# ZhenghaoFei/visual_odom

Measured on NVIDIA H100. Metric: stereo frames/sec at 1241x376, 2000 feats; LK kernel HBM GB/s vs roofline, higher is better.
Workload: dtype u8/i32 fixed point + f32 (LK), f64 (pose)

## Files before the change

### visual_odom_b200/csrc/ctx.cu

```cuda
#include "ctx.h"
#include <string.h>
#include <stdlib.h>

void vo_set_error(vo_ctx* ctx, const char* fmt, ...)
{
    if (!ctx) return;
    va_list ap;
    va_start(ap, fmt);
    vsnprintf(ctx->err, sizeof(ctx->err), fmt, ap);
    va_end(ap);
}

extern "C" void vo_default_params(vo_params* p)
{
    p->fast_threshold = 20;
    p->fast_nonmax = 1;
    p->lk_win = 21;
    p->lk_max_level = 3;
    p->lk_max_iters = 30;
    p->lk_epsilon = 0.01;
    p->lk_min_eig = 0.001;
    p->circ_threshold = 0;
    p->pnp_iterations = 500;
    p->pnp_reproj_error = 0.5f;
// ... 255 lines not shown
}

typedef CUresult (*PFN_cuDeviceGet)(CUdevice*, int);
typedef CUresult (*PFN_cuDeviceGetDevResource)(CUdevice, CUdevResource*, CUdevResourceType);
typedef CUresult (*PFN_cuDevSmResourceSplitByCount)(CUdevResource*, unsigned int*, const CUdevResource*, CUdevResource*, unsigned int, unsigned int);
typedef CUresult (*PFN_cuDevResourceGenerateDesc)(CUdevResourceDesc*, CUdevResource*, unsigned int);
typedef CUresult (*PFN_cuGreenCtxCreate)(CUgreenCtx*, CUdevResourceDesc, CUdevice, unsigned int);
typedef CUresult (*PFN_cuGreenCtxStreamCreate)(CUstream*, CUgreenCtx, unsigned int, int);
typedef CUresult (*PFN_cuGreenCtxDestroy)(CUgreenCtx);

template <typename F>
static bool drv(const char* name, F* fn)
{
    void* p = nullptr;
    cudaDriverEntryPointQueryResult q;
    if (cudaGetDriverEntryPoint(name, &p, cudaEnableDefault, &q) != cudaSuccess || q != cudaDriverEntryPointSuccess || !p) return false;
    *fn = (F)p;
    return true;
}

void vo_partition_destroy(vo_ctx* ctx)
{
    for (auto& L : ctx->lane) {
        if (L.pre) cudaStreamDestroy(L.pre);
        if (L.post && L.post != L.pre) cudaStreamDestroy(L.post);
        L.pre = L.lk = L.post = nullptr;
    }
    PFN_cuGreenCtxDestroy destroy = nullptr;
    if (drv("cuGreenCtxDestroy", &destroy))
        for (int k = 0; k < 2; k++) if (ctx->part_gctx[k]) destroy((CUgreenCtx)ctx->part_gctx[k]);
    ctx->part_gctx[0] = ctx->part_gctx[1] = nullptr;
    ctx->part_on = false; ctx->part_helper_sms = ctx->part_lk_sms = 0;
}

int vo_partition_enable(vo_ctx* ctx, int helper_sms)
{
    VO_CUDA_CHECK(cudaSetDevice(ctx->device));
    int rc = vo_drain_pending(ctx);
    if (rc) return rc;
    VO_CUDA_CHECK(cudaDeviceSynchronize());
    vo_drop_graphs(ctx);
    vo_partition_destroy(ctx);
    if (helper_sms <= 0) return VO_OK;
    PFN_cuDeviceGet dget; PFN_cuDeviceGetDevResource getres; PFN_cuDevSmResourceSplitByCount split;
    PFN_cuDevResourceGenerateDesc gendesc; PFN_cuGreenCtxCreate create; PFN_cuGreenCtxStreamCreate screate;
    if (!drv("cuDeviceGet", &dget) || !drv("cuDeviceGetDevResource", &getres) || !drv("cuDevSmResourceSplitByCount", &split) ||
        !drv("cuDevResourceGenerateDesc", &gendesc) || !drv("cuGreenCtxCreate", &create) || !drv("cuGreenCtxStreamCreate", &screate)) {
        vo_set_error(ctx, "sm_partition: this driver has no green-context API");
        return VO_E_UNSUPPORTED;
    }
    CUdevice dev;
    CUdevResource all, part[1], rest;
    unsigned int nb = 1;
    CUresult r;
    if ((r = dget(&dev, ctx->device)) != CUDA_SUCCESS || (r = getres(dev, &all, CU_DEV_RESOURCE_TYPE_SM)) != CUDA_SUCCESS ||
        (r = split(part, &nb, &all, &rest, 0, (unsigned)helper_sms)) != CUDA_SUCCESS || nb != 1) {
        vo_set_error(ctx, "sm_partition: splitting off %d SMs failed (driver error %d)", helper_sms, (int)r);
        return VO_E_UNSUPPORTED;
    }
    CUdevResource* rs[2] = {&part[0], &rest};
    for (int k = 0; k < 2; k++) {
        CUdevResourceDesc desc;
        CUgreenCtx g;
        if ((r = gendesc(&desc, rs[k], 1)) != CUDA_SUCCESS || (r = create(&g, desc, dev, CU_GREEN_CTX_DEFAULT_STREAM)) != CUDA_SUCCESS) {
            vo_set_error(ctx, "sm_partition: cuGreenCtxCreate failed (driver error %d)", (int)r);
            vo_partition_destroy(ctx);
            return VO_E_UNSUPPORTED;
        }
        ctx->part_gctx[k] = g;
    }
    ctx->part_helper_sms = (int)part[0].sm.smCount; ctx->part_lk_sms = (int)rest.sm.smCount;
    for (int c = 0; c < VO_LANES; c++) {
        CUstream a, b;
        if ((r = screate(&a, (CUgreenCtx)ctx->part_gctx[0], CU_STREAM_NON_BLOCKING, 0)) != CUDA_SUCCESS ||
            (r = screate(&b, (CUgreenCtx)ctx->part_gctx[1], CU_STREAM_NON_BLOCKING, 0)) != CUDA_SUCCESS) {
            vo_set_error(ctx, "sm_partition: cuGreenCtxStreamCreate failed (driver error %d)", (int)r);
            vo_partition_destroy(ctx);
            return VO_E_UNSUPPORTED;
        }
        vo_ctx::Lane& L = ctx->lane[c];
        L.pre = L.lk = (cudaStream_t)b;
        L.post = (cudaStream_t)a;
    }
    ctx->part_on = true;
    return VO_OK;
}

int vo_drain_pending(vo_ctx* ctx)
{
    for (auto& p : ctx->pending)
        if (p.active) {
            VO_CUDA_CHECK(cudaEventSynchronize(p.done));
            p.active = false;
        }
    if (ctx->seq_inflight > 0 && ctx->lane[0].side) VO_CUDA_CHECK(cudaStreamSynchronize(ctx->lane[0].side));
    return VO_OK;
}

void vo_drop_graphs(vo_ctx* ctx)
{
    for (auto& g : ctx->graphs) cudaGraphExecDestroy(g.exec);
    ctx->graphs.clear();
}

static bool same_key(const GraphKey& a, const GraphKey& b)
{
    return a.kind == b.kind && a.s == b.s && a.tma == b.tma && a.u0 == b.u0 && a.n == b.n && a.max_pts == b.max_pts &&
           a.detect == b.detect && a.slot == b.slot && a.parity == b.parity && a.bgr == b.bgr;
}

int vo_run_graph(vo_ctx* ctx, const GraphKey& key, const std::function<int()>& launch)
{
    if (!ctx->use_graphs) return launch();
    for (auto& g : ctx->graphs)
        if (same_key(g.key, key)) {
            VO_CUDA_CHECK(cudaGraphLaunch(g.exec, key.s));
            ctx->launches += g.launches;
            return VO_OK;
        }
    const bool timing = ctx->lk_timing;
    const long long before = ctx->launches;
    ctx->lk_timing = false;
    cudaGraph_t graph = nullptr;
    VO_CUDA_CHECK(cudaStreamBeginCapture(key.s, cudaStreamCaptureModeThreadLocal));
    int rc = launch();
    cudaError_t e = cudaStreamEndCapture(key.s, &graph);
    ctx->lk_timing = timing;
    if (rc) { if (graph) cudaGraphDestroy(graph); return rc; }
    VO_CUDA_CHECK(e);
    vo_ctx::CachedGraph g;
    g.key = key;
    g.launches = ctx->launches - before;
    VO_CUDA_CHECK(cudaGraphInstantiate(&g.exec, graph, 0));
    cudaGraphDestroy(graph);
    ctx->graphs.push_back(g);
    VO_CUDA_CHECK(cudaGraphLaunch(g.exec, key.s));
    return VO_OK;
}

int vo_ensure_lanes(vo_ctx* ctx)
{
    if (ctx->fork_ev) return VO_OK;
    VO_CUDA_CHECK(cudaEventCreateWithFlags(&ctx->fork_ev, cudaEventDisableTiming));
    for (auto& L : ctx->lane) {
        VO_CUDA_CHECK(cudaStreamCreateWithFlags(&L.side, cudaStreamNonBlocking));
        VO_CUDA_CHECK(cudaEventCreateWithFlags(&L.join, cudaEventDisableTiming));
        for (cudaEvent_t& e : L.ev) VO_CUDA_CHECK(cudaEventCreateWithFlags(&e, cudaEventDisableTiming));
    }
    return VO_OK;
}

template <typename T>
static int write_table(vo_ctx* ctx, std::vector<T>& host, T* dev, int u0, int n, const T* e)
{
    const size_t e0 = (size_t)(1 + u0);
    if (memcmp(host.data() + e0, e, n * sizeof(T)) == 0) return VO_OK;
    memcpy(host.data() + e0, e, n * sizeof(T));
    for (auto& p : ctx->pending)
        if (p.active) VO_CUDA_CHECK(cudaStreamWaitEvent(ctx->stream, p.done, 0));
    VO_CUDA_CHECK(cudaMemcpyAsync(dev + e0, host.data() + e0, n * sizeof(T), cudaMemcpyHostToDevice, ctx->stream));
    return VO_OK;
}

int vo_write_calib(vo_ctx* ctx, int u0, int n, const CamCalib* c) { return write_table(ctx, ctx->cal, ctx->d_cal_tab, u0, n, c); }

int vo_write_params(vo_ctx* ctx, int u0, int n, const UnitParams* e) { return write_table(ctx, ctx->par, ctx->d_par_tab, u0, n, e); }

int vo_set_calibration(vo_ctx* ctx, int u0, int n, const float* P_l, const float* P_r, int n_mat)
{
    std::vector<CamCalib> c(n);
    for (int i = 0; i < n; i++) c[i] = vo_calib_from(P_l + 12 * (i % n_mat), P_r + 12 * (i % n_mat));
    return vo_write_calib(ctx, u0, n, c.data());
}

void vo_free_state(vo_ctx* ctx)
{
    vo_drop_graphs(ctx);
    for (void* p : ctx->allocs) cudaFree(p);
    ctx->allocs.clear();
    if (ctx->d_seq_state) cudaFree(ctx->d_seq_state);
    ctx->d_seq_state = nullptr; ctx->seq_n_cap = 0;
    ctx->d_feat_pts = nullptr; ctx->d_feat_ages = nullptr; ctx->d_feat_cnt = ctx->d_bucket = ctx->d_seq_err = ctx->d_seq_live = nullptr;
    ctx->d_out = nullptr; ctx->out_stride = 0; ctx->out_per = 0;
    ctx->d_cal_tab = ctx->d_cal = nullptr;
    ctx->d_par_tab = ctx->d_par = nullptr;
    ctx->d_geo = nullptr;
    ctx->w = ctx->h = ctx->units = 0;
}

template <typename T>
static cudaError_t dalloc(vo_ctx* ctx, T** p, size_t count)
{
    void* q = nullptr;
    cudaError_t e = cudaMalloc(&q, count * sizeof(T) + 256);
    if (e == cudaSuccess) { ctx->allocs.push_back(q); *p = (T*)q; }
    return e;
}

typedef CUresult (*PFN_encodeTiled)(CUtensorMap*, CUtensorMapDataType, cuuint32_t, void*, const cuuint64_t*,
                                    const cuuint64_t*, const cuuint32_t*, const cuuint32_t*, CUtensorMapInterleave,
                                    CUtensorMapSwizzle, CUtensorMapL2promotion, CUtensorMapFloatOOBfill);

static int encode_maps(vo_ctx* ctx)
{
    void* fn = nullptr;
    cudaDriverEntryPointQueryResult qres;
    VO_CUDA_CHECK(cudaGetDriverEntryPoint("cuTensorMapEncodeTiled", &fn, cudaEnableDefault, &qres));
    if (!fn || qres != cudaDriverEntryPointSuccess) {
        vo_set_error(ctx, "cuTensorMapEncodeTiled not available from the driver");
        return VO_E_CUDA;
    }
    PFN_encodeTiled enc = (PFN_encodeTiled)fn;
    const int n_img = ctx->units * 4;
    for (int l = 0; l < ctx->pg.nlevels; l++) {
        const LevelGeom& g = ctx->pg.lv[l];
        {
            cuuint64_t dims[3] = {(cuuint64_t)g.pitch, (cuuint64_t)g.hp, (cuuint64_t)n_img};
            cuuint64_t strides[2] = {(cuuint64_t)g.pitch, (cuuint64_t)g.plane};
            cuuint32_t box_i[3] = {48, 22, 1}, box_j[3] = {48, 32, 1};
            cuuint32_t estr[3] = {1, 1, 1};
            CUresult r = enc(&ctx->maps.img_i[l], CU_TENSOR_MAP_DATA_TYPE_UINT8, 3, g.img, dims, strides, box_i, estr,
                             CU_TENSOR_MAP_INTERLEAVE_NONE, CU_TENSOR_MAP_SWIZZLE_NONE,
                             CU_TENSOR_MAP_L2_PROMOTION_NONE, CU_TENSOR_MAP_FLOAT_OOB_FILL_NONE);
            if (r == CUDA_SUCCESS)
                r = enc(&ctx->maps.img_j[l], CU_TENSOR_MAP_DATA_TYPE_UINT8, 3, g.img, dims, strides, box_j, estr,
                        CU_TENSOR_MAP_INTERLEAVE_NONE, CU_TENSOR_MAP_SWIZZLE_NONE,
                        CU_TENSOR_MAP_L2_PROMOTION_NONE, CU_TENSOR_MAP_FLOAT_OOB_FILL_NONE);
            if (r != CUDA_SUCCESS) { vo_set_error(ctx, "cuTensorMapEncodeTiled(u8 level %d) failed: %d", l, (int)r); return VO_E_CUDA; }
        }
        {
            cuuint64_t dims[3] = {(cuuint64_t)g.pitch, (cuuint64_t)g.hp, (cuuint64_t)n_img};
            cuuint64_t strides[2] = {(cuuint64_t)g.pitch * 4, (cuuint64_t)g.plane * 4};
            cuuint32_t box[3] = {28, 22, 1};
            cuuint32_t estr[3] = {1, 1, 1};
            CUresult r = enc(&ctx->maps.der[l], CU_TENSOR_MAP_DATA_TYPE_UINT32, 3, g.der, dims, strides, box, estr,
                             CU_TENSOR_MAP_INTERLEAVE_NONE, CU_TENSOR_MAP_SWIZZLE_NONE,
                             CU_TENSOR_MAP_L2_PROMOTION_NONE, CU_TENSOR_MAP_FLOAT_OOB_FILL_NONE);
            if (r != CUDA_SUCCESS) { vo_set_error(ctx, "cuTensorMapEncodeTiled(deriv level %d) failed: %d", l, (int)r); return VO_E_CUDA; }
        }
    }
    return VO_OK;
}

int vo_ensure_state(vo_ctx* ctx, int w, int h, int units, int levels)
{
    if (w <= 0 || h <= 0 || units <= 0) { vo_set_error(ctx, "bad geometry %dx%d units=%d", w, h, units); return VO_E_INVALID; }
    const int depth = vo_pyr_depth(w, h, ctx->p.lk_max_level);
    if (levels <= 0 || levels > depth) levels = depth;
    if (ctx->w == w && ctx->h == h && ctx->units >= units && ctx->pg.nlevels == levels) return VO_OK;
    VO_CUDA_CHECK(cudaSetDevice(ctx->device));
    { int drc = vo_drain_pending(ctx); if (drc) return drc; }
    VO_CUDA_CHECK(cudaStreamSynchronize(ctx->stream));
    vo_free_state(ctx);
    const int n_img = units * 4;
    const int cap = ctx->cap;
    PyrGeom& pg = ctx->pg;
    memset(&pg, 0, sizeof(pg));
    int cw = w, ch = h;
    for (int l = 0; l < levels; l++) {
        if (l > 0) { cw = (cw + 1) / 2; ch = (ch + 1) / 2; }
        LevelGeom& g = pg.lv[l];
        g.w = cw; g.h = ch;
        g.pitch = ((cw + 2 * VO_PAD) + 63) / 64 * 64;
        g.hp = ch + 2 * VO_PAD;
        g.plane = (size_t)g.pitch * g.hp;
        VO_CUDA_CHECK(dalloc(ctx, &g.img, g.plane * n_img));
        VO_CUDA_CHECK(dalloc(ctx, &g.der, g.plane * n_img));
        VO_CUDA_CHECK(cudaMemsetAsync(g.img, 0, g.plane * n_img, ctx->stream));
        VO_CUDA_CHECK(cudaMemsetAsync(g.der, 0, g.plane * n_img * sizeof(uint32_t), ctx->stream));
        pg.nlevels = l + 1;
    }
    pg.n_img = n_img;
    VO_CUDA_CHECK(dalloc(ctx, &ctx->d_raw, (size_t)n_img * w * h));
    VO_CUDA_CHECK(dalloc(ctx, &ctx->d_raw_tab, (size_t)n_img));
    VO_CUDA_CHECK(dalloc(ctx, &ctx->d_ingest_tab, (size_t)n_img));
    {
        std::vector<const uint8_t*> tab(n_img);
        for (int i = 0; i < n_img; i++) tab[i] = ctx->d_raw + (size_t)i * w * h;
        VO_CUDA_CHECK(cudaMemcpyAsync(ctx->d_raw_tab, tab.data(), n_img * sizeof(uint8_t*), cudaMemcpyHostToDevice, ctx->stream));
        VO_CUDA_CHECK(cudaStreamSynchronize(ctx->stream));
    }
    const size_t uc = (size_t)units * cap;
    VO_CUDA_CHECK(dalloc(ctx, &ctx->d_pts_in, uc));
    VO_CUDA_CHECK(dalloc(ctx, &ctx->d_npts, (size_t)units));
    VO_CUDA_CHECK(dalloc(ctx, &ctx->d_pts_out, 4 * uc));
    VO_CUDA_CHECK(dalloc(ctx, &ctx->d_status, 4 * uc));
    VO_CUDA_CHECK(dalloc(ctx, &ctx->d_err, 4 * uc));
    VO_CUDA_CHECK(dalloc(ctx, &ctx->d_lk_progress, uc));
    VO_CUDA_CHECK(cudaMemsetAsync(ctx->d_lk_progress, 0, uc * sizeof(int), ctx->stream));
    VO_CUDA_CHECK(dalloc(ctx, &ctx->d_ages_in, uc));
    VO_CUDA_CHECK(dalloc(ctx, &ctx->d_ages_out, uc));
    VO_CUDA_CHECK(dalloc(ctx, &ctx->d_kept5, 5 * uc));
    VO_CUDA_CHECK(dalloc(ctx, &ctx->d_idx3, uc));
    VO_CUDA_CHECK(dalloc(ctx, &ctx->d_n3, (size_t)units));
    VO_CUDA_CHECK(dalloc(ctx, &ctx->d_valid4, 4 * uc));
    VO_CUDA_CHECK(dalloc(ctx, &ctx->d_idx5, uc));
    VO_CUDA_CHECK(dalloc(ctx, &ctx->d_n5, (size_t)units));
    {
        const long iw = w > 6 ? w - 6 : 0, ih = h > 6 ? h - 6 : 0;
        const long bound = ctx->p.fast_nonmax ? ((iw + 1) / 2) * ((ih + 1) / 2) : iw * ih;
        if (bound > (1L << 30)) { vo_set_error(ctx, "%dx%d: too many possible FAST corners", w, h); return VO_E_CAPACITY; }
        ctx->corner_cap = bound > 0 ? (int)bound : 1;
    }
    VO_CUDA_CHECK(dalloc(ctx, &ctx->d_score, (size_t)units * w * h));
    VO_CUDA_CHECK(dalloc(ctx, &ctx->d_rowbuf, (size_t)units * h * w));
    VO_CUDA_CHECK(dalloc(ctx, &ctx->d_rowcount, (size_t)units * h));
    VO_CUDA_CHECK(dalloc(ctx, &ctx->d_rowoff, (size_t)units * h));
    VO_CUDA_CHECK(dalloc(ctx, &ctx->d_ndet, (size_t)units));
    VO_CUDA_CHECK(dalloc(ctx, &ctx->d_corners, (size_t)units * ctx->corner_cap));
    VO_CUDA_CHECK(dalloc(ctx, &ctx->d_resp, (size_t)units * ctx->corner_cap));
    VO_CUDA_CHECK(dalloc(ctx, &ctx->d_want, (size_t)units));
    const size_t its = (size_t)vo_pnp_iterations(ctx);
    VO_CUDA_CHECK(dalloc(ctx, &ctx->d_X, uc));
    VO_CUDA_CHECK(dalloc(ctx, &ctx->d_tprev, (size_t)units * 3));
    VO_CUDA_CHECK(dalloc(ctx, &ctx->d_pnp_state, (size_t)units));
    VO_CUDA_CHECK(dalloc(ctx, &ctx->d_subsets, (size_t)units * its * 5));
    VO_CUDA_CHECK(dalloc(ctx, &ctx->d_models, (size_t)units * its * 12));
    VO_CUDA_CHECK(dalloc(ctx, &ctx->d_counts, (size_t)units * its));
    VO_CUDA_CHECK(dalloc(ctx, &ctx->d_inliers, uc));
    VO_CUDA_CHECK(dalloc(ctx, &ctx->d_results, (size_t)units));
    VO_CUDA_CHECK(dalloc(ctx, &ctx->d_cal_tab, 1 + (size_t)units));
    ctx->d_cal = ctx->d_cal_tab + 1;
    ctx->cal.resize(1 + (size_t)units, CamCalib{});
    VO_CUDA_CHECK(cudaMemcpyAsync(ctx->d_cal_tab, ctx->cal.data(), (1 + (size_t)units) * sizeof(CamCalib), cudaMemcpyHostToDevice, ctx->stream));
    VO_CUDA_CHECK(dalloc(ctx, &ctx->d_par_tab, 1 + (size_t)units));
    ctx->d_par = ctx->d_par_tab + 1;
    ctx->par.resize(1 + (size_t)units, vo_unit_params(ctx->p));
    VO_CUDA_CHECK(cudaMemcpyAsync(ctx->d_par_tab, ctx->par.data(), (1 + (size_t)units) * sizeof(UnitParams), cudaMemcpyHostToDevice, ctx->stream));
    ctx->feat_cap = ctx->corner_cap + cap;
    ctx->seq_active = false;
    VO_CUDA_CHECK(cudaMemsetAsync(ctx->d_results, 0, (size_t)units * sizeof(vo_unit_result_dev), ctx->stream));
    VO_CUDA_CHECK(cudaMemsetAsync(ctx->d_tprev, 0, (size_t)units * 3 * sizeof(double), ctx->stream));
    ctx->w = w; ctx->h = h; ctx->units = units;
    VO_CUDA_CHECK(dalloc(ctx, &ctx->d_geo, (size_t)n_img));
    ctx->geo.assign((size_t)n_img, vo_plane_geom(ctx, w, h));
    VO_CUDA_CHECK(cudaMemcpyAsync(ctx->d_geo, ctx->geo.data(), (size_t)n_img * sizeof(PlaneGeom), cudaMemcpyHostToDevice, ctx->stream));
    int rc = encode_maps(ctx);
    if (rc != VO_OK) { vo_free_state(ctx); return rc; }
    VO_CUDA_CHECK(cudaStreamSynchronize(ctx->stream));
    return VO_OK;
}

PlaneGeom vo_plane_geom(const vo_ctx* ctx, int w, int h)
{
    PlaneGeom g;
    memset(&g, 0, sizeof(g));
    for (int l = 0; l < ctx->pg.nlevels; l++) {
        g.w[l] = w; g.h[l] = h;
        w = (w + 1) / 2; h = (h + 1) / 2;
    }
    g.pitch = g.w[0];
    return g;
}

int vo_write_geo(vo_ctx* ctx, int p0, int n, const PlaneGeom* g, cudaStream_t st)
{
    if (memcmp(ctx->geo.data() + p0, g, n * sizeof(PlaneGeom)) == 0) return VO_OK;
    memcpy(ctx->geo.data() + p0, g, n * sizeof(PlaneGeom));
    VO_CUDA_CHECK(cudaMemcpyAsync(ctx->d_geo + p0, ctx->geo.data() + p0, n * sizeof(PlaneGeom), cudaMemcpyHostToDevice,
                                  st ? st : ctx->stream));
    return VO_OK;
}

int vo_run_pyramid(vo_ctx* ctx, int plane0, int nplanes, cudaStream_t s, bool sized)
{
    PyrGeom pg = ctx->pg;
    pg.n_img = nplanes;
    for (int l = 0; l < pg.nlevels; l++) {
        pg.lv[l].img += (size_t)plane0 * pg.lv[l].plane;
        pg.lv[l].der += (size_t)plane0 * pg.lv[l].plane;
    }
    ctx->launches += vo_launch_pyramid(pg, ctx->d_raw_tab + plane0, ctx->w, sized ? ctx->d_geo + plane0 : nullptr, s);
    VO_CUDA_CHECK(cudaGetLastError());
    return VO_OK;
}

int vo_run_lk(vo_ctx* ctx, const View& v, int ncalls, const int* img_prev, const int* img_next, bool want_err, const UnitParams* par)
{
    int rc = vo_run_pyramid(ctx, v.u0 * v.imgs, v.n * v.imgs, v.s);
    if (rc) return rc;
    return vo_run_lk_ring(ctx, v, ncalls, img_prev, img_next, want_err, par);
}

int vo_run_lk_ring(vo_ctx* ctx, const View& v, int ncalls, const int* img_prev, const int* img_next, bool want_err,
                   const UnitParams* par)
{
    const size_t uo = (size_t)v.u0 * ctx->cap;
    const PyrGeom& pg = ctx->pg;

    LkArgs a;
    memset(&a, 0, sizeof(a));
    a.n_units = v.n;
    a.cap = ctx->cap;
    a.n_pts = ctx->d_npts + v.u0;
    a.imgs_per_unit = v.imgs;
    a.img_plane0 = v.plane0 >= 0 ? v.plane0 : v.u0 * v.imgs;
    a.ncalls = ncalls;
    for (int c = 0; c < ncalls; c++) { a.img_prev[c] = img_prev[c]; a.img_next[c] = img_next[c]; }
    a.nlevels = pg.nlevels;
    for (int l = 0; l < pg.nlevels; l++) { a.lw[l] = pg.lv[l].w; a.lh[l] = pg.lv[l].h; }
    a.geo = v.sized ? ctx->d_geo : nullptr;
    a.par = par + v.u0;
    a.pts_in = ctx->d_pts_in + uo;
    a.pts_out = ctx->d_pts_out + uo;
    a.status_out = ctx->d_status + uo;
    a.err_out = want_err ? ctx->d_err + uo : nullptr;
    a.call_stride = (size_t)ctx->units * ctx->cap;
    a.use_tma = ctx->lk_use_tma ? 1 : 0;
    for (int l = 0; l < pg.nlevels; l++) {
        a.img_base[l] = ctx->pg.lv[l].img; a.der_base[l] = ctx->pg.lv[l].der;
        a.pitch[l] = pg.lv[l].pitch; a.plane[l] = pg.lv[l].plane;
    }

    cudaEvent_t e0 = nullptr, e1 = nullptr;
    if (ctx->lk_timing) {
        if (ctx->ev_used + 2 > ctx->ev_pool.size()) {
            cudaEvent_t a0, a1;
            VO_CUDA_CHECK(cudaEventCreate(&a0));
            VO_CUDA_CHECK(cudaEventCreate(&a1));
            ctx->ev_pool.push_back(a0); ctx->ev_pool.push_back(a1);
        }
        e0 = ctx->ev_pool[ctx->ev_used]; e1 = ctx->ev_pool[ctx->ev_used + 1];
        ctx->ev_used += 2;
        VO_CUDA_CHECK(cudaEventRecord(e0, v.s));
    }
    {
        size_t qi = 0;
        while (qi < ctx->lk_queue_streams.size() && ctx->lk_queue_streams[qi] != v.s) qi++;
        if (qi == ctx->lk_queue_streams.size()) {
            if (qi >= LK_QUEUES) { vo_set_error(ctx, "more than %d streams launch the LK kernel", LK_QUEUES); return VO_E_CAPACITY; }
            ctx->lk_queue_streams.push_back(v.s);
        }
        a.queue = ctx->d_lk_queue + 2 * qi;
        a.per_unit = v.max_pts > 0 && v.max_pts < ctx->cap ? v.max_pts : ctx->cap;
        a.progress = ctx->d_lk_progress + uo;
        int lk_sms = ctx->sm_count;
        for (const auto& L : ctx->lane) if (ctx->part_on && v.s == L.lk) lk_sms = ctx->part_lk_sms;
        const bool big = (long)a.n_units * a.per_unit > (long)lk_sms * LK_CTAS_PER_SM * LK_WARPS_PER_CTA;
        a.span = ctx->lk_span > 0 ? ctx->lk_span : (big ? 2 : 0);
        VO_CUDA_CHECK(vo_launch_lk_ring(ctx->maps, a, lk_sms, v.s));
    }
    ctx->launches += 1;
    if (e1) VO_CUDA_CHECK(cudaEventRecord(e1, v.s));
    return VO_OK;
}

int vo_run_filter(vo_ctx* ctx, const View& v, bool with_ages, const UnitParams* par)
{
    const size_t uo = (size_t)v.u0 * ctx->cap;
    FilterArgs f;
    memset(&f, 0, sizeof(f));
    f.cap = ctx->cap;
    f.call_stride = (size_t)ctx->units * ctx->cap;
    f.par = par + v.u0;
    f.n_pts = ctx->d_npts + v.u0;
    f.pts_in = ctx->d_pts_in + uo;
    f.pts_out = ctx->d_pts_out + uo;
    f.status = ctx->d_status + uo;
    f.ages_in = with_ages ? ctx->d_ages_in + uo : nullptr;
    f.ages_out = ctx->d_ages_out + uo;
    f.kept5 = ctx->d_kept5 + uo;
    f.idx3 = ctx->d_idx3 + uo;
    f.n3 = ctx->d_n3 + v.u0;
    f.valid4 = ctx->d_valid4 + uo;
    f.idx5 = ctx->d_idx5 + uo;
    f.n5 = ctx->d_n5 + v.u0;
    VO_CUDA_CHECK(vo_launch_ring_filter(f, v.n, v.s));
    ctx->launches += 1;
    return VO_OK;
}

int vo_run_fast(vo_ctx* ctx, const View& v, int plane_in_unit, bool want_resp, const UnitParams* par)
{
    FastArgs a;
    memset(&a, 0, sizeof(a));
    const size_t plane = (size_t)ctx->w * ctx->h;
    a.n_units = v.n;
    a.img_tab = ctx->d_raw_tab + (size_t)(v.plane0 >= 0 ? v.plane0 : v.u0 * v.imgs) + plane_in_unit;
    a.img_stride_idx = v.imgs;
    a.w = ctx->w; a.h = ctx->h; a.pitch = ctx->w;
    a.par = par + v.u0; a.nonmax = ctx->p.fast_nonmax;
    a.score = ctx->d_score + v.u0 * plane; a.score_plane = plane;
    a.rowbuf = ctx->d_rowbuf + v.u0 * plane; a.rowcap = ctx->w;
    a.rowcount = ctx->d_rowcount + (size_t)v.u0 * ctx->h; a.rowoff = ctx->d_rowoff + (size_t)v.u0 * ctx->h;
    a.n_det = ctx->d_ndet + v.u0;
    a.corners = ctx->d_corners + (size_t)v.u0 * ctx->corner_cap;
    a.resp = want_resp ? ctx->d_resp + (size_t)v.u0 * ctx->corner_cap : nullptr;
    a.corner_cap = ctx->corner_cap;
    a.geo = v.sized ? ctx->d_geo + (a.img_tab - ctx->d_raw_tab) : nullptr;
    ctx->launches += vo_launch_fast(a, v.s);
    VO_CUDA_CHECK(cudaGetLastError());
    return VO_OK;
}

int vo_run_select(vo_ctx* ctx, const View& v)
{
    ctx->launches += vo_launch_select(ctx->d_corners + (size_t)v.u0 * ctx->corner_cap, ctx->corner_cap, ctx->d_ndet + v.u0,
                                      ctx->d_want + v.u0, ctx->d_pts_in + (size_t)v.u0 * ctx->cap, ctx->cap, ctx->d_npts + v.u0,
                                      v.n, v.s);
    VO_CUDA_CHECK(cudaGetLastError());
    return VO_OK;
}

int vo_run_triangulate(vo_ctx* ctx, const View& v, const float2* pts_l, const float2* pts_r, const int* n, const CamCalib* cal,
                       float4* X4)
{
    const size_t uo = (size_t)v.u0 * ctx->cap;
    TriArgs t;
    memset(&t, 0, sizeof(t));
    t.cap = ctx->cap; t.n_pts = n + v.u0; t.pts_l = pts_l + uo; t.pts_r = pts_r + uo; t.X = ctx->d_X + uo; t.X4 = X4;
    t.cal = cal + v.u0;
    ctx->launches += vo_launch_triangulate(t, v.n, v.s);
    VO_CUDA_CHECK(cudaGetLastError());
    return VO_OK;
}

int vo_run_pnp(vo_ctx* ctx, const View& v, const float2* pts2d, const int* n, const CamCalib* cal, const UnitParams* par)
{
    const int iterations = vo_pnp_iterations(ctx);
    const size_t uo = (size_t)v.u0 * ctx->cap, its = (size_t)iterations;
    PnpArgs a;
    memset(&a, 0, sizeof(a));
    a.n_units = v.n; a.cap = ctx->cap; a.iterations = iterations;
    a.n_pts = n + v.u0; a.X = ctx->d_X + uo; a.x = pts2d + uo;
    a.cal = cal + v.u0;
    a.par = par + v.u0;
    a.t_prev = ctx->d_tprev + (size_t)v.u0 * 3;
    a.state = ctx->d_pnp_state + v.u0; a.subsets = ctx->d_subsets + v.u0 * its * 5; a.models = ctx->d_models + v.u0 * its * 12;
    a.counts = ctx->d_counts + v.u0 * its;
    a.inliers = ctx->d_inliers + uo; a.results = ctx->d_results + v.u0;
    ctx->launches += vo_launch_pnp(a, v.s);
    VO_CUDA_CHECK(cudaGetLastError());
    return VO_OK;
}
```

### visual_odom_b200/csrc/fast.cu

```cuda
#include "common.cuh"
#include "fast.h"

__global__ void __launch_bounds__(256) k_fast_score(const uint8_t* const* __restrict__ img_tab, int img_stride_idx,
                                                    int w, int h, int pitch, const UnitParams* __restrict__ par, int nonmax,
                                                    uint8_t* __restrict__ score, size_t score_plane,
                                                    const PlaneGeom* __restrict__ geo)
{
    constexpr int ring_dx[16] = {0, 1, 2, 3, 3, 3, 2, 1, 0, -1, -2, -3, -3, -3, -2, -1};
    constexpr int ring_dy[16] = {3, 3, 2, 1, 0, -1, -2, -3, -3, -3, -2, -1, 0, 1, 2, 3};
    const int unit = blockIdx.z;
    const int threshold = par[unit].fast_threshold;
    const uint8_t* __restrict__ img = img_tab[unit * img_stride_idx];
    uint8_t* __restrict__ sc = score + (size_t)unit * score_plane;
    if (geo) { const PlaneGeom& g = geo[unit * img_stride_idx]; w = g.w[0]; h = g.h[0]; pitch = g.pitch; }
    const int x = blockIdx.x * 32 + (threadIdx.x & 31);
    const int y = blockIdx.y * 8 + (threadIdx.x >> 5);
    if (x >= w || y >= h) return;
    int result = 0;
    if (x >= 3 && x < w - 3 && y >= 3 && y < h - 3) {
        const uint8_t* p = img + (size_t)y * pitch + x;
        const int v = p[0];
        float d[16];
        unsigned hi = 0, lo = 0;
#pragma unroll
        for (int k = 0; k < 16; k++) {
            const int r = p[ring_dy[k] * pitch + ring_dx[k]];
            d[k] = (float)(v - r);
            hi |= (unsigned)(r > v + threshold) << k;
            lo |= (unsigned)(r < v - threshold) << k;
        }
        unsigned mh = hi | (hi << 16), ml = lo | (lo << 16);
        mh &= mh >> 1; mh &= mh >> 2; mh &= mh >> 4; mh &= mh >> 1;
        ml &= ml >> 1; ml &= ml >> 2; ml &= ml >> 4; ml &= ml >> 1;
        if (mh | ml) {
            float mn[16], mx[16];
#pragma unroll
            for (int k = 0; k < 16; k++) { mn[k] = fminf(d[k], d[(k + 1) & 15]); mx[k] = fmaxf(d[k], d[(k + 1) & 15]); }
            float mn4[16], mx4[16];
#pragma unroll
            for (int k = 0; k < 16; k++) { mn4[k] = fminf(mn[k], mn[(k + 2) & 15]); mx4[k] = fmaxf(mx[k], mx[(k + 2) & 15]); }
            float A = -1000.f, B = 1000.f;
#pragma unroll
            for (int k = 0; k < 16; k++) {
                const float a8 = fminf(mn4[k], mn4[(k + 4) & 15]);
                const float b8 = fmaxf(mx4[k], mx4[(k + 4) & 15]);
                A = fmaxf(A, fminf(a8, d[(k + 8) & 15]));
                B = fminf(B, fmaxf(b8, d[(k + 8) & 15]));
            }
            result = max(threshold, (int)fmaxf(A, -B)) - 1;
            if (!nonmax) result = 1;
        }
    }
    sc[(size_t)y * w + x] = (uint8_t)result;
}

#define NMS_T 256
#define NMS_NC 8
__global__ void __launch_bounds__(NMS_T) k_fast_nms_row(const uint8_t* __restrict__ score, size_t score_plane, int w, int h,
                                                        int nonmax, uint16_t* __restrict__ rowbuf, int rowcap,
                                                        int* __restrict__ rowcount, const PlaneGeom* __restrict__ geo,
                                                        int geo_stride)
{
    const int y = blockIdx.x, unit = blockIdx.y;
    int iw = w, ih = h;
    if (geo) { iw = geo[unit * geo_stride].w[0]; ih = geo[unit * geo_stride].h[0]; }
    const uint8_t* __restrict__ sc = score + (size_t)unit * score_plane;
    uint16_t* __restrict__ out = rowbuf + ((size_t)unit * h + y) * rowcap;
    __shared__ uint8_t rows[3][NMS_T * NMS_NC + 2];
    __shared__ int wcnt[NMS_NC * (NMS_T / 32)];
    __shared__ int base;
    if (y < 3 || y >= ih - 3) {
        if (threadIdx.x == 0) rowcount[unit * h + y] = 0;
        return;
    }
    if (threadIdx.x == 0) base = 0;
    const int lane = threadIdx.x & 31, warp = threadIdx.x >> 5;
    constexpr int NW = NMS_T / 32, SPAN = NMS_T * NMS_NC;
    for (int x0 = 0; x0 < iw; x0 += SPAN) {
        for (int i = threadIdx.x; i < SPAN + 2; i += NMS_T) {
            const int x = x0 - 1 + i;
            const bool in = (x >= 0 && x < iw);
            rows[0][i] = in ? sc[(size_t)(y - 1) * iw + x] : 0;
            rows[1][i] = in ? sc[(size_t)y * iw + x] : 0;
            rows[2][i] = in ? sc[(size_t)(y + 1) * iw + x] : 0;
        }
        __syncthreads();
        unsigned bal[NMS_NC];
#pragma unroll
        for (int c = 0; c < NMS_NC; c++) {
            const int x = x0 + c * NMS_T + threadIdx.x, i = c * NMS_T + threadIdx.x + 1;
            bool keep = false;
            if (x < iw) {
                const int s = rows[1][i];
                if (s > 0) {
                    keep = !nonmax ||
                           (s > rows[1][i - 1] && s > rows[1][i + 1] && s > rows[0][i - 1] && s > rows[0][i] &&
                            s > rows[0][i + 1] && s > rows[2][i - 1] && s > rows[2][i] && s > rows[2][i + 1]);
                }
            }
            bal[c] = __ballot_sync(0xffffffffu, keep);
            if (lane == 0) wcnt[c * NW + warp] = __popc(bal[c]);
        }
        __syncthreads();
        int carry_total = 0;
        if (threadIdx.x < NMS_NC * NW) {
            const int v = wcnt[threadIdx.x];
            int incl = v;
#pragma unroll
            for (int d = 1; d < 32; d <<= 1) {
                const int o = __shfl_up_sync(0xffffffffu, incl, d);
                if (lane >= d) incl += o;
            }
            carry_total = incl;
            wcnt[threadIdx.x] = incl - v;
        }
        __shared__ int w0_total, pass_total;
        if (threadIdx.x == 31) w0_total = carry_total;
        __syncthreads();
        if (threadIdx.x >= 32 && threadIdx.x < NMS_NC * NW) wcnt[threadIdx.x] += w0_total;
        if (threadIdx.x == NMS_NC * NW - 1) pass_total = carry_total + w0_total;
        __syncthreads();
        const int b0 = base;
#pragma unroll
        for (int c = 0; c < NMS_NC; c++) {
            if ((bal[c] >> lane) & 1u) {
                const int o = b0 + wcnt[c * NW + warp] + __popc(bal[c] & ((1u << lane) - 1u));
                if (o < rowcap) out[o] = (uint16_t)(x0 + c * NMS_T + threadIdx.x);
            }
        }
        __syncthreads();
        if (threadIdx.x == 0) base = b0 + pass_total;
        __syncthreads();
    }
    if (threadIdx.x == 0) rowcount[unit * h + y] = base < rowcap ? base : rowcap;
}

__global__ void __launch_bounds__(1024) k_fast_scan(const int* __restrict__ rowcount, int h, int* __restrict__ rowoff,
                                                    int* __restrict__ n_det)
{
    const int unit = blockIdx.x;
    const int* rc = rowcount + unit * h;
    int* ro = rowoff + unit * h;
    __shared__ int wsum[32];
    __shared__ int carry;
    if (threadIdx.x == 0) carry = 0;
    __syncthreads();
    const int lane = threadIdx.x & 31, warp = threadIdx.x >> 5;
    for (int y0 = 0; y0 < h; y0 += 1024) {
        const int y = y0 + threadIdx.x;
        int v = (y < h) ? rc[y] : 0;
        int incl = v;
#pragma unroll
        for (int d = 1; d < 32; d <<= 1) {
            int o = __shfl_up_sync(0xffffffffu, incl, d);
            if (lane >= d) incl += o;
        }
        if (lane == 31) wsum[warp] = incl;
        __syncthreads();
        int woff = carry;
        for (int k = 0; k < warp; k++) woff += wsum[k];
        if (y < h) ro[y] = woff + incl - v;
        __syncthreads();
        if (threadIdx.x == 0) {
            int t = 0;
            for (int k = 0; k < 32; k++) t += wsum[k];
            carry += t;
        }
        __syncthreads();
    }
    if (threadIdx.x == 0) n_det[unit] = carry;
}

__global__ void __launch_bounds__(128) k_fast_gather(const uint16_t* __restrict__ rowbuf, int rowcap,
                                                     const int* __restrict__ rowcount, const int* __restrict__ rowoff,
                                                     int h, const uint8_t* __restrict__ score, size_t score_plane, int w,
                                                     int nonmax, float2* __restrict__ out, float* __restrict__ resp, int cap,
                                                     const PlaneGeom* __restrict__ geo, int geo_stride)
{
    const int y = blockIdx.x, unit = blockIdx.y;
    if (geo) w = geo[unit * geo_stride].w[0];
    const int n = rowcount[unit * h + y], off = rowoff[unit * h + y];
    const uint16_t* src = rowbuf + ((size_t)unit * h + y) * rowcap;
    for (int i = threadIdx.x; i < n; i += blockDim.x) {
        const int o = off + i;
        if (o < cap) {
            const int x = src[i];
            out[(size_t)unit * cap + o] = make_float2((float)x, (float)y);
            if (resp)
                resp[(size_t)unit * cap + o] = nonmax ? (float)score[(size_t)unit * score_plane + (size_t)y * w + x] : 0.f;
        }
    }
}

__global__ void k_select_stride(const float2* __restrict__ corners, int corner_cap, const int* __restrict__ n_det,
                                const int* __restrict__ want, float2* __restrict__ pts, int cap, int* __restrict__ n_pts)
{
    const int unit = blockIdx.y;
    int m = n_det[unit];
    if (m > corner_cap) m = corner_cap;
    int n = want[unit];
    if (n > cap) n = cap;
    if (n > m) n = m;
    const int i = blockIdx.x * blockDim.x + threadIdx.x;
    if (i == 0) n_pts[unit] = n;
    if (i >= n) return;
    const long idx = (n > 1) ? ((long)i * (m - 1)) / (n - 1) : 0;
    pts[(size_t)unit * cap + i] = corners[(size_t)unit * corner_cap + idx];
}

int vo_launch_fast(const FastArgs& a, cudaStream_t stream)
{
    dim3 g1((a.w + 31) / 32, (a.h + 7) / 8, a.n_units);
    k_fast_score<<<g1, 256, 0, stream>>>(a.img_tab, a.img_stride_idx, a.w, a.h, a.pitch, a.par, a.nonmax, a.score,
                                          a.score_plane, a.geo);
    dim3 g2(a.h, a.n_units);
    k_fast_nms_row<<<g2, NMS_T, 0, stream>>>(a.score, a.score_plane, a.w, a.h, a.nonmax, a.rowbuf, a.rowcap, a.rowcount, a.geo,
                                              a.img_stride_idx);
    k_fast_scan<<<a.n_units, 1024, 0, stream>>>(a.rowcount, a.h, a.rowoff, a.n_det);
    k_fast_gather<<<g2, 128, 0, stream>>>(a.rowbuf, a.rowcap, a.rowcount, a.rowoff, a.h, a.score, a.score_plane, a.w,
                                           a.nonmax, a.corners, a.resp, a.corner_cap, a.geo, a.img_stride_idx);
    return 4;
}

int vo_launch_select(const float2* corners, int corner_cap, const int* n_det, const int* want, float2* pts, int cap,
                     int* n_pts, int n_units, cudaStream_t stream)
{
    dim3 g((cap + 255) / 256, n_units);
    k_select_stride<<<g, 256, 0, stream>>>(corners, corner_cap, n_det, want, pts, cap, n_pts);
    return 1;
}
```

### visual_odom_b200/csrc/fast.h

```cpp
#pragma once
#include "common.cuh"

struct FastArgs {
    int n_units;
    const uint8_t* const* img_tab;
    int img_stride_idx;
    int w, h, pitch;
    const UnitParams* par;
    int nonmax;
    uint8_t* score;
    size_t score_plane;
    uint16_t* rowbuf;
    int rowcap;
    int* rowcount;
    int* rowoff;
    int* n_det;
    float2* corners;
    float* resp;
    int corner_cap;
    const PlaneGeom* geo;
};

int vo_launch_fast(const FastArgs& a, cudaStream_t stream);
int vo_launch_select(const float2* corners, int corner_cap, const int* n_det, const int* want, float2* pts, int cap,
                     int* n_pts, int n_units, cudaStream_t stream);
```

Measured before the change: 4116.

## Rewrite FAST scoring and NMS with shared-memory tiles and SIMD byte ops

FAST scoring now stages a 128x32 image tile (plus halo) in shared memory and tests four pixels per thread using packed byte SIMD compares. The full corner score is computed only for compacted candidates, and results are written as 32-bit words into a 4-byte-aligned pitched score buffer. NMS now processes four rows per block with packed byte max ops and ballot-based compaction instead of per-pixel scalar loads and block-wide scans. This is meant to cut redundant global loads and per-pixel work in the detector, in exchange for more complex indexing and a new score pitch that every consumer must use consistently.

Result: faster. 4183, median of 6 (+1.6%).

```diff
diff --git a/visual_odom_b200/csrc/ctx.cu b/visual_odom_b200/csrc/ctx.cu
--- a/visual_odom_b200/csrc/ctx.cu
+++ b/visual_odom_b200/csrc/ctx.cu
@@ -581,7 +581,7 @@
         if (bound > (1L << 30)) { vo_set_error(ctx, "%dx%d: too many possible FAST corners", w, h); return VO_E_CAPACITY; }
         ctx->corner_cap = bound > 0 ? (int)bound : 1;
     }
-    VO_CUDA_CHECK(dalloc(ctx, &ctx->d_score, (size_t)units * w * h));
+    VO_CUDA_CHECK(dalloc(ctx, &ctx->d_score, (size_t)units * vo_fast_score_pitch(w) * h));
     VO_CUDA_CHECK(dalloc(ctx, &ctx->d_rowbuf, (size_t)units * h * w));
     VO_CUDA_CHECK(dalloc(ctx, &ctx->d_rowcount, (size_t)units * h));
     VO_CUDA_CHECK(dalloc(ctx, &ctx->d_rowoff, (size_t)units * h));
@@ -759,7 +759,8 @@
     a.img_stride_idx = v.imgs;
     a.w = ctx->w; a.h = ctx->h; a.pitch = ctx->w;
     a.par = par + v.u0; a.nonmax = ctx->p.fast_nonmax;
-    a.score = ctx->d_score + v.u0 * plane; a.score_plane = plane;
+    const size_t score_plane = (size_t)vo_fast_score_pitch(ctx->w) * ctx->h;
+    a.score = ctx->d_score + v.u0 * score_plane; a.score_plane = score_plane;
     a.rowbuf = ctx->d_rowbuf + v.u0 * plane; a.rowcap = ctx->w;
     a.rowcount = ctx->d_rowcount + (size_t)v.u0 * ctx->h; a.rowoff = ctx->d_rowoff + (size_t)v.u0 * ctx->h;
     a.n_det = ctx->d_ndet + v.u0;
diff --git a/visual_odom_b200/csrc/fast.cu b/visual_odom_b200/csrc/fast.cu
--- a/visual_odom_b200/csrc/fast.cu
+++ b/visual_odom_b200/csrc/fast.cu
@@ -1,38 +1,124 @@
 #include "common.cuh"
 #include "fast.h"
 
+
+#define FS_TW 128
+#define FS_TH 32
+#define FS_SW (FS_TW / 4 + 2)
+#define FS_SR (FS_TH + 6)
+
+static __device__ __forceinline__ uint32_t fs_bytes(const uint32_t* wr, int dx)
+{
+    return dx < 0 ? __funnelshift_r(wr[0], wr[1], 8 * (4 + dx)) : dx == 0 ? wr[1] : __funnelshift_r(wr[1], wr[2], 8 * dx);
+}
+
+static __device__ __forceinline__ bool fs_arc9(uint32_t m)
+{
+    m &= m >> 1; m &= m >> 2; m &= m >> 4; m &= m >> 1;
+    return m != 0;
+}
+
 __global__ void __launch_bounds__(256) k_fast_score(const uint8_t* const* __restrict__ img_tab, int img_stride_idx,
                                                     int w, int h, int pitch, const UnitParams* __restrict__ par, int nonmax,
-                                                    uint8_t* __restrict__ score, size_t score_plane,
+                                                    uint8_t* __restrict__ score, size_t score_plane, int score_pitch,
                                                     const PlaneGeom* __restrict__ geo)
 {
     constexpr int ring_dx[16] = {0, 1, 2, 3, 3, 3, 2, 1, 0, -1, -2, -3, -3, -3, -2, -1};
     constexpr int ring_dy[16] = {3, 3, 2, 1, 0, -1, -2, -3, -3, -3, -2, -1, 0, 1, 2, 3};
+    __shared__ uint32_t tile[FS_SR][FS_SW];
+    __shared__ uint32_t sco[FS_TH][FS_TW / 4];
+    __shared__ uint16_t cand[FS_TH * FS_TW];
+    __shared__ int ncand;
     const int unit = blockIdx.z;
     const int threshold = par[unit].fast_threshold;
     const uint8_t* __restrict__ img = img_tab[unit * img_stride_idx];
     uint8_t* __restrict__ sc = score + (size_t)unit * score_plane;
     if (geo) { const PlaneGeom& g = geo[unit * img_stride_idx]; w = g.w[0]; h = g.h[0]; pitch = g.pitch; }
-    const int x = blockIdx.x * 32 + (threadIdx.x & 31);
-    const int y = blockIdx.y * 8 + (threadIdx.x >> 5);
-    if (x >= w || y >= h) return;
-    int result = 0;
-    if (x >= 3 && x < w - 3 && y >= 3 && y < h - 3) {
-        const uint8_t* p = img + (size_t)y * pitch + x;
-        const int v = p[0];
-        float d[16];
-        unsigned hi = 0, lo = 0;
-#pragma unroll
-        for (int k = 0; k < 16; k++) {
-            const int r = p[ring_dy[k] * pitch + ring_dx[k]];
-            d[k] = (float)(v - r);
-            hi |= (unsigned)(r > v + threshold) << k;
-            lo |= (unsigned)(r < v - threshold) << k;
-        }
-        unsigned mh = hi | (hi << 16), ml = lo | (lo << 16);
-        mh &= mh >> 1; mh &= mh >> 2; mh &= mh >> 4; mh &= mh >> 1;
-        ml &= ml >> 1; ml &= ml >> 2; ml &= ml >> 4; ml &= ml >> 1;
-        if (mh | ml) {
+    const int x0 = blockIdx.x * FS_TW, y0 = blockIdx.y * FS_TH;
+    if (x0 >= w || y0 >= h) return;
+    if (threadIdx.x == 0) ncand = 0;
+
+    constexpr int FS_K = (FS_SR * FS_SW + 255) / 256;
+    uint32_t staged[FS_K];
+#pragma unroll
+    for (int k = 0; k < FS_K; k++) {
+        const int i = threadIdx.x + 256 * k;
+        const int r = i / FS_SW, j = i - r * FS_SW, y = y0 - 3 + r;
+        uint32_t lo = 0, hi = 0;
+        unsigned sh = 0;
+        if (i < FS_SR * FS_SW && y >= 0 && y < h) {
+            const uintptr_t rb = (uintptr_t)(img + (size_t)y * pitch), re = rb + (uintptr_t)w;
+            const uintptr_t a = rb + (intptr_t)(x0 - 4 + 4 * j), a0 = a & ~(uintptr_t)3;
+            sh = (unsigned)(a & 3) * 8;
+            if (a0 < re && a0 + 4 > rb) lo = __ldg(reinterpret_cast<const uint32_t*>(a0));
+            if (sh && a0 + 4 < re && a0 + 8 > rb) hi = __ldg(reinterpret_cast<const uint32_t*>(a0 + 4));
+        }
+        staged[k] = __funnelshift_r(lo, hi, sh);
+    }
+#pragma unroll
+    for (int k = 0; k < FS_K; k++) {
+        const int i = threadIdx.x + 256 * k;
+        if (i < FS_SR * FS_SW) (&tile[0][0])[i] = staged[k];
+    }
+    __syncthreads();
+
+    const int lane = threadIdx.x & 31, warp = threadIdx.x >> 5;
+    const int x = x0 + 4 * lane;
+    const uint32_t t4 = (uint32_t)threshold * 0x01010101u;
+    uint32_t cbits = 0;
+#pragma unroll
+    for (int k = 0; k < 4; k++) {
+        const int ly = warp * 4 + k, y = y0 + ly;
+        const uint32_t c = tile[ly + 3][lane + 1];
+        const uint32_t cp = __vaddus4(c, t4), cm = __vsubus4(c, t4);
+        uint32_t ha = 0, hb = 0, la = 0, lb = 0;
+#pragma unroll
+        for (int q = 0; q < 16; q++) {
+            const uint32_t r = fs_bytes(&tile[ly + 3 + ring_dy[q]][lane], ring_dx[q]);
+            const uint32_t bit = 0x01010101u << (q & 7);
+            const uint32_t g = __vcmpgtu4(r, cp) & bit, l = __vcmpltu4(r, cm) & bit;
+            if (q < 8) { ha |= g; la |= l; } else { hb |= g; lb |= l; }
+        }
+        uint32_t rb = 0;
+#pragma unroll
+        for (int i = 0; i < 4; i++) {
+            const uint32_t sel = i | (4 + i) << 4 | i << 8 | (4 + i) << 12;
+            const bool inner = x + i >= 3 && x + i < w - 3 && y >= 3 && y < h - 3;
+            if (inner && (fs_arc9(__byte_perm(ha, hb, sel)) || fs_arc9(__byte_perm(la, lb, sel)))) rb |= 1u << i;
+        }
+        cbits |= rb << (4 * k);
+        sco[ly][lane] = nonmax ? 0u : (rb * 0x00204081u) & 0x01010101u;
+    }
+
+    if (nonmax) {
+        const int n = __popc(cbits);
+        int incl = n;
+#pragma unroll
+        for (int d = 1; d < 32; d <<= 1) {
+            const int o = __shfl_up_sync(0xffffffffu, incl, d);
+            if (lane >= d) incl += o;
+        }
+        int base = 0;
+        if (lane == 31 && incl) base = atomicAdd(&ncand, incl);
+        int o = __shfl_sync(0xffffffffu, base, 31) + incl - n;
+        for (uint32_t b = cbits; b; b &= b - 1) {
+            const int bit = __ffs(b) - 1;
+            cand[o++] = (uint16_t)((warp * 4 + (bit >> 2)) * FS_TW + 4 * lane + (bit & 3));
+        }
+    }
+    __syncthreads();
+
+    if (nonmax) {
+        const uint8_t* tb = reinterpret_cast<const uint8_t*>(tile);
+        uint8_t* sb = reinterpret_cast<uint8_t*>(sco);
+        const int nc = ncand;
+        for (int i = threadIdx.x; i < nc; i += blockDim.x) {
+            const int e = cand[i], ly = e / FS_TW, lx = e - ly * FS_TW;
+            const uint8_t* p = tb + (ly + 3) * (FS_SW * 4) + lx + 4;
+            const int v = p[0];
+            float d[16];
+#pragma unroll
+            for (int k = 0; k < 16; k++) d[k] = (float)(v - (int)p[ring_dy[k] * (FS_SW * 4) + ring_dx[k]]);
             float mn[16], mx[16];
 #pragma unroll
             for (int k = 0; k < 16; k++) { mn[k] = fminf(d[k], d[(k + 1) & 15]); mx[k] = fmaxf(d[k], d[(k + 1) & 15]); }
@@ -47,92 +133,84 @@
                 A = fmaxf(A, fminf(a8, d[(k + 8) & 15]));
                 B = fminf(B, fmaxf(b8, d[(k + 8) & 15]));
             }
-            result = max(threshold, (int)fmaxf(A, -B)) - 1;
-            if (!nonmax) result = 1;
-        }
-    }
-    sc[(size_t)y * w + x] = (uint8_t)result;
-}
-
-#define NMS_T 256
-#define NMS_NC 8
-__global__ void __launch_bounds__(NMS_T) k_fast_nms_row(const uint8_t* __restrict__ score, size_t score_plane, int w, int h,
-                                                        int nonmax, uint16_t* __restrict__ rowbuf, int rowcap,
-                                                        int* __restrict__ rowcount, const PlaneGeom* __restrict__ geo,
-                                                        int geo_stride)
-{
-    const int y = blockIdx.x, unit = blockIdx.y;
+            sb[ly * FS_TW + lx] = (uint8_t)(max(threshold, (int)fmaxf(A, -B)) - 1);
+        }
+        __syncthreads();
+    }
+
+    for (int i = threadIdx.x; i < FS_TH * (FS_TW / 4); i += blockDim.x) {
+        const int r = i / (FS_TW / 4), j = i - r * (FS_TW / 4), y = y0 + r, xw = x0 + 4 * j;
+        if (y < h && xw < w) *reinterpret_cast<uint32_t*>(sc + (size_t)y * score_pitch + xw) = sco[r][j];
+    }
+}
+
+#define NMS_R 4
+#define NMS_SPAN 2048
+#define NMS_SW (NMS_SPAN / 4 + 2)
+__global__ void __launch_bounds__(NMS_R * 32) k_fast_nms_row(const uint8_t* __restrict__ score, size_t score_plane,
+                                                             int score_pitch, int w, int h, int nonmax,
+                                                             uint16_t* __restrict__ rowbuf, int rowcap,
+                                                             int* __restrict__ rowcount, const PlaneGeom* __restrict__ geo,
+                                                             int geo_stride)
+{
+    __shared__ uint32_t rows[NMS_R + 2][NMS_SW];
+    const int unit = blockIdx.y, y0 = blockIdx.x * NMS_R;
     int iw = w, ih = h;
     if (geo) { iw = geo[unit * geo_stride].w[0]; ih = geo[unit * geo_stride].h[0]; }
     const uint8_t* __restrict__ sc = score + (size_t)unit * score_plane;
+    const int lane = threadIdx.x & 31, warp = threadIdx.x >> 5, y = y0 + warp;
+    const bool live = y >= 3 && y < ih - 3;
     uint16_t* __restrict__ out = rowbuf + ((size_t)unit * h + y) * rowcap;
-    __shared__ uint8_t rows[3][NMS_T * NMS_NC + 2];
-    __shared__ int wcnt[NMS_NC * (NMS_T / 32)];
-    __shared__ int base;
-    if (y < 3 || y >= ih - 3) {
-        if (threadIdx.x == 0) rowcount[unit * h + y] = 0;
-        return;
-    }
-    if (threadIdx.x == 0) base = 0;
-    const int lane = threadIdx.x & 31, warp = threadIdx.x >> 5;
-    constexpr int NW = NMS_T / 32, SPAN = NMS_T * NMS_NC;
-    for (int x0 = 0; x0 < iw; x0 += SPAN) {
-        for (int i = threadIdx.x; i < SPAN + 2; i += NMS_T) {
-            const int x = x0 - 1 + i;
-            const bool in = (x >= 0 && x < iw);
-            rows[0][i] = in ? sc[(size_t)(y - 1) * iw + x] : 0;
-            rows[1][i] = in ? sc[(size_t)y * iw + x] : 0;
-            rows[2][i] = in ? sc[(size_t)(y + 1) * iw + x] : 0;
-        }
-        __syncthreads();
-        unsigned bal[NMS_NC];
-#pragma unroll
-        for (int c = 0; c < NMS_NC; c++) {
-            const int x = x0 + c * NMS_T + threadIdx.x, i = c * NMS_T + threadIdx.x + 1;
-            bool keep = false;
-            if (x < iw) {
-                const int s = rows[1][i];
-                if (s > 0) {
-                    keep = !nonmax ||
-                           (s > rows[1][i - 1] && s > rows[1][i + 1] && s > rows[0][i - 1] && s > rows[0][i] &&
-                            s > rows[0][i + 1] && s > rows[2][i - 1] && s > rows[2][i] && s > rows[2][i + 1]);
+    const unsigned lt = (1u << lane) - 1u;
+    int base = 0;
+    for (int x0 = 0; x0 < iw; x0 += NMS_SPAN) {
+        __syncthreads();
+        constexpr int NMS_K = ((NMS_R + 2) * NMS_SW + NMS_R * 32 - 1) / (NMS_R * 32);
+        uint32_t staged[NMS_K];
+#pragma unroll
+        for (int k = 0; k < NMS_K; k++) {
+            const int i = threadIdx.x + NMS_R * 32 * k;
+            const int r = i / NMS_SW, j = i - r * NMS_SW, yy = y0 - 1 + r, xx = x0 - 4 + 4 * j;
+            staged[k] = (i < (NMS_R + 2) * NMS_SW && yy >= 0 && yy < ih && xx >= 0 && xx < iw)
+                            ? __ldg(reinterpret_cast<const uint32_t*>(sc + (size_t)yy * score_pitch + xx)) : 0u;
+        }
+#pragma unroll
+        for (int k = 0; k < NMS_K; k++) {
+            const int i = threadIdx.x + NMS_R * 32 * k;
+            if (i < (NMS_R + 2) * NMS_SW) (&rows[0][0])[i] = staged[k];
+        }
+        __syncthreads();
+        if (!live) continue;
+        for (int c = 0; c < NMS_SPAN / 128 && x0 + c * 128 < iw; c++) {
+            const uint32_t* t = &rows[warp][c * 32 + lane];
+            const uint32_t* m = &rows[warp + 1][c * 32 + lane];
+            const uint32_t* b = &rows[warp + 2][c * 32 + lane];
+            const uint32_t s = m[1];
+            uint32_t keep;
+            if (nonmax) {
+                const uint32_t nt = __vmaxu4(__vmaxu4(fs_bytes(t, -1), t[1]), fs_bytes(t, 1));
+                const uint32_t nb = __vmaxu4(__vmaxu4(fs_bytes(b, -1), b[1]), fs_bytes(b, 1));
+                const uint32_t nm = __vmaxu4(fs_bytes(m, -1), fs_bytes(m, 1));
+                keep = __vcmpgtu4(s, __vmaxu4(__vmaxu4(nt, nb), nm));
+            } else {
+                keep = __vcmpgtu4(s, 0u);
+            }
+            const unsigned b0 = __ballot_sync(0xffffffffu, keep & 0x000000ffu);
+            const unsigned b1 = __ballot_sync(0xffffffffu, keep & 0x0000ff00u);
+            const unsigned b2 = __ballot_sync(0xffffffffu, keep & 0x00ff0000u);
+            const unsigned b3 = __ballot_sync(0xffffffffu, keep & 0xff000000u);
+            int o = base + __popc(b0 & lt) + __popc(b1 & lt) + __popc(b2 & lt) + __popc(b3 & lt);
+            const int x = x0 + c * 128 + 4 * lane;
+#pragma unroll
+            for (int i = 0; i < 4; i++)
+                if (keep & (0xffu << (8 * i))) {
+                    if (o < rowcap) out[o] = (uint16_t)(x + i);
+                    o++;
                 }
-            }
-            bal[c] = __ballot_sync(0xffffffffu, keep);
-            if (lane == 0) wcnt[c * NW + warp] = __popc(bal[c]);
-        }
-        __syncthreads();
-        int carry_total = 0;
-        if (threadIdx.x < NMS_NC * NW) {
-            const int v = wcnt[threadIdx.x];
-            int incl = v;
-#pragma unroll
-            for (int d = 1; d < 32; d <<= 1) {
-                const int o = __shfl_up_sync(0xffffffffu, incl, d);
-                if (lane >= d) incl += o;
-            }
-            carry_total = incl;
-            wcnt[threadIdx.x] = incl - v;
-        }
-        __shared__ int w0_total, pass_total;
-        if (threadIdx.x == 31) w0_total = carry_total;
-        __syncthreads();
-        if (threadIdx.x >= 32 && threadIdx.x < NMS_NC * NW) wcnt[threadIdx.x] += w0_total;
-        if (threadIdx.x == NMS_NC * NW - 1) pass_total = carry_total + w0_total;
-        __syncthreads();
-        const int b0 = base;
-#pragma unroll
-        for (int c = 0; c < NMS_NC; c++) {
-            if ((bal[c] >> lane) & 1u) {
-                const int o = b0 + wcnt[c * NW + warp] + __popc(bal[c] & ((1u << lane) - 1u));
-                if (o < rowcap) out[o] = (uint16_t)(x0 + c * NMS_T + threadIdx.x);
-            }
-        }
-        __syncthreads();
-        if (threadIdx.x == 0) base = b0 + pass_total;
-        __syncthreads();
-    }
-    if (threadIdx.x == 0) rowcount[unit * h + y] = base < rowcap ? base : rowcap;
+            base += __popc(b0) + __popc(b1) + __popc(b2) + __popc(b3);
+        }
+    }
+    if (lane == 0 && y < h) rowcount[unit * h + y] = !live ? 0 : base < rowcap ? base : rowcap;
 }
 
 __global__ void __launch_bounds__(1024) k_fast_scan(const int* __restrict__ rowcount, int h, int* __restrict__ rowoff,
@@ -173,12 +251,11 @@
 
 __global__ void __launch_bounds__(128) k_fast_gather(const uint16_t* __restrict__ rowbuf, int rowcap,
                                                      const int* __restrict__ rowcount, const int* __restrict__ rowoff,
-                                                     int h, const uint8_t* __restrict__ score, size_t score_plane, int w,
-                                                     int nonmax, float2* __restrict__ out, float* __restrict__ resp, int cap,
-                                                     const PlaneGeom* __restrict__ geo, int geo_stride)
+                                                     int h, const uint8_t* __restrict__ score, size_t score_plane,
+                                                     int score_pitch, int nonmax, float2* __restrict__ out,
+                                                     float* __restrict__ resp, int cap)
 {
     const int y = blockIdx.x, unit = blockIdx.y;
-    if (geo) w = geo[unit * geo_stride].w[0];
     const int n = rowcount[unit * h + y], off = rowoff[unit * h + y];
     const uint16_t* src = rowbuf + ((size_t)unit * h + y) * rowcap;
     for (int i = threadIdx.x; i < n; i += blockDim.x) {
@@ -187,7 +264,7 @@
             const int x = src[i];
             out[(size_t)unit * cap + o] = make_float2((float)x, (float)y);
             if (resp)
-                resp[(size_t)unit * cap + o] = nonmax ? (float)score[(size_t)unit * score_plane + (size_t)y * w + x] : 0.f;
+                resp[(size_t)unit * cap + o] = nonmax ? (float)score[(size_t)unit * score_plane + (size_t)y * score_pitch + x] : 0.f;
         }
     }
 }
@@ -210,15 +287,17 @@
 
 int vo_launch_fast(const FastArgs& a, cudaStream_t stream)
 {
-    dim3 g1((a.w + 31) / 32, (a.h + 7) / 8, a.n_units);
+    const int sp = vo_fast_score_pitch(a.w);
+    dim3 g1((a.w + FS_TW - 1) / FS_TW, (a.h + FS_TH - 1) / FS_TH, a.n_units);
     k_fast_score<<<g1, 256, 0, stream>>>(a.img_tab, a.img_stride_idx, a.w, a.h, a.pitch, a.par, a.nonmax, a.score,
-                                          a.score_plane, a.geo);
-    dim3 g2(a.h, a.n_units);
-    k_fast_nms_row<<<g2, NMS_T, 0, stream>>>(a.score, a.score_plane, a.w, a.h, a.nonmax, a.rowbuf, a.rowcap, a.rowcount, a.geo,
-                                              a.img_stride_idx);
+                                          a.score_plane, sp, a.geo);
+    dim3 g2((a.h + NMS_R - 1) / NMS_R, a.n_units);
+    k_fast_nms_row<<<g2, NMS_R * 32, 0, stream>>>(a.score, a.score_plane, sp, a.w, a.h, a.nonmax, a.rowbuf, a.rowcap,
+                                                   a.rowcount, a.geo, a.img_stride_idx);
     k_fast_scan<<<a.n_units, 1024, 0, stream>>>(a.rowcount, a.h, a.rowoff, a.n_det);
-    k_fast_gather<<<g2, 128, 0, stream>>>(a.rowbuf, a.rowcap, a.rowcount, a.rowoff, a.h, a.score, a.score_plane, a.w,
-                                           a.nonmax, a.corners, a.resp, a.corner_cap, a.geo, a.img_stride_idx);
+    dim3 g3(a.h, a.n_units);
+    k_fast_gather<<<g3, 128, 0, stream>>>(a.rowbuf, a.rowcap, a.rowcount, a.rowoff, a.h, a.score, a.score_plane, sp,
+                                           a.nonmax, a.corners, a.resp, a.corner_cap);
     return 4;
 }
 
diff --git a/visual_odom_b200/csrc/fast.h b/visual_odom_b200/csrc/fast.h
--- a/visual_odom_b200/csrc/fast.h
+++ b/visual_odom_b200/csrc/fast.h
@@ -21,6 +21,8 @@
     const PlaneGeom* geo;
 };
 
+static inline int vo_fast_score_pitch(int w) { return (w + 3) & ~3; }
+
 int vo_launch_fast(const FastArgs& a, cudaStream_t stream);
 int vo_launch_select(const float2* corners, int corner_cap, const int* n_det, const int* want, float2* pts, int cap,
                      int* n_pts, int n_units, cudaStream_t stream);
```
